# GlassyWing/yolo_deepsort

Hardware: AMD Instinct MI355X
Metric: end-to-end frames/sec (detect+ReID+assoc), 608x608 (higher is better)
Workload: dtype f16x3

## Files before the change

### include/ydsort.h

```cpp
#ifndef YDSORT_H
#define YDSORT_H

#include <stddef.h>
#include <stdint.h>

#ifdef __cplusplus
extern "C" {
#endif

typedef struct yds_net yds_net;
typedef struct yds_reid yds_reid;
typedef struct yds_trk yds_trk;
typedef struct yds_pipe yds_pipe;
typedef struct yds_comm yds_comm;

int yds_init(int device_id);
int yds_current_device(void);
int yds_device_pci_bus_id(char *buf, int len);
const char *yds_last_error(void);
int yds_device_count(void);
const char *yds_build_info(void);
void *yds_host_alloc(size_t nbytes);
int yds_host_free(void *host);
void *yds_dev_alloc(size_t nbytes);
// ... 39 lines not shown

yds_reid *yds_reid_create(int max_crops);
void yds_reid_destroy(yds_reid *);
int yds_reid_load_tensor(yds_reid *, const char *name, const float *data_host, const int64_t *shape, int ndim);
int yds_reid_finalize(yds_reid *);
int64_t yds_reid_flops_per_crop(void);
int yds_reid_embed(yds_reid *, const uint8_t *frame_rgb_host, int h, int w, const float *tlwh_host,
                   int D, float *out_host);
int yds_reid_embed_dev(yds_reid *, const uint8_t *frame_rgb_dev, int h, int w, const float *tlwh_host,
                       int D, float *out_host_or_null);
const float *yds_reid_features_dev(yds_reid *);
int yds_reid_preprocess(yds_reid *, const uint8_t *frame_rgb_host, int h, int w, const float *tlwh_host,
                        int D, float *nchw_host);
int yds_reid_preprocess_mixed(yds_reid *, const uint8_t *frames_rgb_dev, const uint64_t *frame_off, const int32_t *frame_hw ,
                              int n_frames, size_t frames_bytes, const float *tlwh_host, const int32_t *frame_of_host, int D, float *nchw_host);
int yds_reid_forward_f32(yds_reid *, const float *nchw_host, int D, float *out_host);

yds_trk *yds_tracker_create(double max_dist, double max_iou_distance, int max_age, int n_init, int nn_budget);
yds_trk *yds_tracker_create_ex(double max_dist, double max_iou_distance, int max_age, int n_init, int nn_budget, int metric);
void yds_tracker_destroy(yds_trk *);
int yds_tracker_step(yds_trk *, const float *tlwh_host, const float *feats_host, const float *payload_host,
                     int D, int32_t *out6_host, int cap, int *m_out,
                     int32_t *dbg_matches_host, int dbg_cap, int *n_matches);
int yds_tracker_step_dev(yds_trk *, const float *tlwh_host, const float *feats_dev, const float *payload_host,
                         int D, int32_t *out6_host, int cap, int *m_out);
int yds_tracker_step_sel(yds_trk *, const float *tlwh_host, const float *feats, int feats_on_device, const int32_t *feat_rows_host,
                         const float *payload_host, int D, int32_t *out6_host, int cap, int *m_out,
                         int32_t *dbg_matches_host, int dbg_cap, int *n_matches);
int yds_tracker_nms(const float *tlwh_host, const int32_t *order_host, int D, double max_overlap, int32_t *pick_host, int *n_pick);
int yds_tracker_num_tracks(const yds_trk *);
// ... 94 lines not shown
```

### yolo_deepsort_amd/_lib.py

```python

from __future__ import annotations

import ctypes as C
import os

import numpy as np

HERE = os.path.dirname(os.path.abspath(__file__))
_TAG = os.environ.get("YDS_BUILD_TAG", "")
LIB_PATH = os.path.join(HERE, "libydsort" + ("_" + _TAG if _TAG else "") + ".so")


class YdsError(RuntimeError):
    pass


_P = C.c_void_p
_I = C.c_int
_F = C.c_float
_SZ = C.c_size_t
_I64 = C.c_int64

SIGNATURES = {
    "yds_init": (_I, [_I]),
# ... 99 lines not shown
    "yds_pipeline_step_multi_host": (_I, [_P, _P, _P, _I, _I, _I, _P, _P, _I, _P]),
    "yds_pipeline_prefetch_host": (_I, [_P, _P, _I, _I, _I]),
    "yds_pipeline_set_next_injection": (_I, [_P, _I]),
    "yds_pipeline_stage_us": (_I, [_P, _P]),
    "yds_pipeline_set_schedule": (_I, [_P, _I]),
    "yds_pipeline_last_schedule": (_I, [_P]),
    "yds_pipeline_schedule_trial": (_I, [_P, _I, _P, _P, _P]),
    "yds_conv_timing": (_I, [_P, _I, _P, _P, _P]),
    "yds_overlay_tracks": (_I, [_P, _P, _I, _I, _I, _P, _P, _P, _I, _P, _P, _I, _I, _I, _P, _P]),
    "yds_swap_rb": (_I, [_P, _SZ]),
    "yds_overlay_tracks_bgr": (_I, [_P, _I, _P, _I, _I, _I, _P, _P, _P, _I, _P, _P, _I, _I, _I, _P]),
    "yds_pipeline_set_frame_order": (_I, [_P, _I]),
    "yds_pipeline_set_windows": (_I, [_P, _I, _I, C.c_double]),
    "yds_darknet_forward_u8_mixed_dev": (_I, [_P, _P, _P, _P, _SZ, _I]),
    "yds_reid_preprocess_mixed": (_I, [_P, _P, _P, _P, _I, _SZ, _P, _P, _I, _P]),
    "yds_pipeline_step_multi_mixed": (_I, [_P, _P, _P, _P, _P, _SZ, _I, _P, _P, _I, _P]),
    "yds_pipeline_step_multi_mixed_host": (_I, [_P, _P, _P, _P, _P, _SZ, _I, _P, _P, _I, _P]),
}

_lib = None
MISSING = []


def load():
    global _lib
    if _lib is not None:
        return _lib
    if not os.path.exists(LIB_PATH):
        raise YdsError(f"{LIB_PATH} not found: build it with `python -m yolo_deepsort_amd.build` "
                       "(the product has no CPU fallback)")
# ... 138 lines not shown
```

### yolo_deepsort_amd/csrc/common.h

```cpp
#pragma once
#include <hip/hip_runtime.h>
#include <stdint.h>
#include <stdio.h>
#include <string>
#include <vector>
#include <stdexcept>

namespace yds {

void set_error(const std::string &msg);
struct Error : std::runtime_error {
    explicit Error(const std::string &m) : std::runtime_error(m) {}
};
[[noreturn]] void fail(const char *fmt, ...);
int bound_device();
void bind_thread();
hipStream_t make_stream(bool latency_role);

#define YDS_HIP(expr)                                                                          \
    do {                                                                                       \
        hipError_t _e = (expr);                                                                \
        if (_e != hipSuccess)                                                                  \
            ::yds::fail("%s failed: %s (%s:%d)", #expr, hipGetErrorString(_e), __FILE__, __LINE__); \
    } while (0)
// ... 97 lines not shown
                   float logit, hipStream_t s);
void launch_inject_batch(const View &head, int batch, const float *table_dev, const int *offsets_dev, int max_rows, int head_index,
                         int num_classes, float logit, hipStream_t s);
void launch_resize_u8(const uint8_t *frames, int n, int h, int w, const View &y, hipStream_t s, bool bgr = false);
struct FrameGeom { uint64_t off; int32_t h, w; };
std::vector<FrameGeom> checked_layout(const uint64_t *frame_off, const int32_t *frame_hw, int n, size_t frames_bytes);
void launch_resize_u8_frames(const uint8_t *frames, const FrameGeom *geom, int n, const View &y, hipStream_t s, bool bgr = false);
void launch_window_resize(const uint8_t *frames, int h, int w, const int *tiles_dev, int T, int slot0, int n, const View &y, hipStream_t s,
                          bool bgr);
void launch_window_boxes(const float *pred, int n_boxes, int attrs, const int *tiles_dev, const float *scale_dev, int T, int slot0, int n,
                         float *dst, hipStream_t s);
void launch_crop_resize(const uint8_t *frames, int h, int w, const int *boxes5_dev, int D, const View &y,
                        hipStream_t s, bool bgr = false);
void launch_crop_resize_frames(const uint8_t *frames, const FrameGeom *geom, const int *boxes5_dev, int D, const View &y, hipStream_t s,
                               bool bgr = false);
void launch_avgpool_l2norm(const View &x, float *out, hipStream_t s);

}
```

### yolo_deepsort_amd/csrc/engine.h

```cpp
#pragma once
#include "common.h"

#include <map>
#include <memory>
#include <string>
#include <utility>
#include <vector>

namespace yds {

struct CfgBlock {
    std::string type;
    std::map<std::string, std::string> kv;
};
std::vector<CfgBlock> parse_cfg(const std::string &text);

struct Layer {
    std::string type;
    int c = 0, h = 0, w = 0;
    int root = -1, coff = 0;
    bool is_view = false;
    int src = -1;
    std::vector<int> refs;
    std::vector<std::pair<int, int>> copies;
// ... 138 lines not shown
    DevBuf<float> kept;
    DevBuf<int> order;
    int *h_counts = nullptr;
    float *h_kept = nullptr;
};

class ReidNet {
public:
    explicit ReidNet(int max_crops);
    ~ReidNet();
    void load_tensor(const std::string &name, const float *data, const int64_t *shape, int ndim);
    void finalize();
    void embed_dev(const uint8_t *frame_dev, int h, int w, const float *tlwh_host, int D, float *out_host);
    void embed_multi_dev(const uint8_t *frames_dev, int h, int w, const float *tlwh_host, const int *frame_of, int D, bool bgr = false,
                         const FrameGeom *geom = nullptr, int n_geom = 0);
    void crop_multi_dev(const uint8_t *frames_dev, int h, int w, const float *tlwh_host, const int *frame_of, int D, bool bgr,
                        const FrameGeom *geom, int n_geom);
    void preprocess_frames_dev(const uint8_t *frames_dev, const std::vector<FrameGeom> &geom, const float *tlwh_host, const int *frame_of, int D,
                               float *nchw_host);
    void embed_host(const uint8_t *frame_host, int h, int w, const float *tlwh_host, int D, float *out_host);
    void preprocess_host(const uint8_t *frame_host, int h, int w, const float *tlwh_host, int D, float *nchw_host);
    void forward_f32_host(const float *nchw, int D, float *out_host);
    void forward(int D);
    void reserve(int D);
    void allocate_buffers();
    static int64_t flops_per_crop();

    struct ConvW {
        int cin = 0, cin_file = 0, cout = 0, k = 0, stride = 1, pad = 0, kpad = 0;
        DevBuf<float> wt, bias;
        DevBuf<uint16_t> wt16;
    };
    int max_crops;
    std::map<std::string, std::vector<float>> raw;
    std::map<std::string, std::vector<int64_t>> raw_shape;
    bool ready = false;
    std::vector<ConvW> convs;
    std::vector<DevBuf<float>> bufs;
    DevBuf<float> in, feat, stage_f32;
    DevBuf<uint8_t> stage_u8;
    DevBuf<int> boxes_dev;
    std::vector<int> boxes_host;
    int *boxes_pin[2] = {nullptr, nullptr};
    size_t boxes_pin_cap[2] = {0, 0};
    int boxes_pin_turn = 0;
    hipStream_t sync_before_regrow = nullptr;
    std::map<int, std::pair<int, int>> tuned;
    int tuned_math = -1;
    hipStream_t stream = nullptr;
    double conv_flops_last = 0;
};

struct TrackerIface {
    virtual ~TrackerIface() {}
    virtual int step(const float *tlwh_host, const float *feats, bool feats_on_device, const float *payload_host, int D,
                     int32_t *out6_host, int cap) = 0;
    virtual int num_tracks() const = 0;
};
struct TrackerGroupIface {
    virtual ~TrackerGroupIface() {}
    virtual void step_batch(TrackerIface *const *trk, int S, int n, const int *stream_of, const float *tlwh_host, const int *first,
                            const float *feats_dev, const float *payload_host, const char *skip, int32_t *out6_host, int cap, int32_t *counts) = 0;
    virtual void wait_for(hipEvent_t ev) = 0;
};
TrackerGroupIface *make_tracker_group();
// ... 7 lines not shown
```

### yolo_deepsort_amd/csrc/layers.hip

```cpp
#include "common.h"

#include <algorithm>
#include "h16.h"

namespace yds {

static inline int grid_for(size_t work, int block = 256) {
    size_t g = (work + block - 1) / block;
    if (g > 8192) g = 8192;
    if (g < 1) g = 1;
    return (int)g;
}

__global__ void maxpool_kernel(const float *x, float *y, int N, int H, int W, int C, int ldx, int Ho, int Wo, int ldy,
                               int k, int stride, int pad, int zero_br, int fmt_in, int fmt_out) {
    fp16_saturate_on();
    const int C4 = C >> 2;
    const size_t total = (size_t)N * Ho * Wo * C4;
    for (size_t idx = blockIdx.x * (size_t)blockDim.x + threadIdx.x; idx < total; idx += (size_t)gridDim.x * blockDim.x) {
        int c4 = idx % C4;
        size_t pix = idx / C4;
        int ox = pix % Wo;
        size_t t = pix / Wo;
        int oy = t % Ho;
// ... 278 lines not shown
        else v = (t - 5 == cls) ? logit : -logit;
        cell[t] = v;
    }
}
void launch_inject_batch(const View &head, int batch, const float *table_dev, const int *offsets_dev, int max_rows, int head_index,
                         int num_classes, float logit, hipStream_t s) {
    int attrs = num_classes + 5, A = head.c / attrs;
    hipLaunchKernelGGL(inject_clear_batch_kernel, dim3(min(grid_for((size_t)head.h * head.w * A), 64), batch), dim3(256), 0, s, head.p, head.h,
                       head.w, head.ld, A, attrs, logit);
    if (max_rows > 0)
        hipLaunchKernelGGL(inject_rows_batch_kernel, dim3(max_rows, batch), dim3(128), 0, s, head.p, head.h, head.w, head.ld, attrs, table_dev,
                           offsets_dev, head_index, logit);
    YDS_HIP(hipGetLastError());
}

struct Tap { int i0, i1, a0, a1; };
__device__ __forceinline__ double cv_scale(int dst, int src) { return __ddiv_rn(1.0, __ddiv_rn((double)dst, (double)src)); }
template <bool X_AXIS> __device__ __forceinline__ Tap axis_tap(int d, double scale, int src) {
    float f = __double2float_rn(__dsub_rn(__dmul_rn((double)d + 0.5, scale), 0.5));
    const float fl = floorf(f);
    int s = (int)fl;
    f = __fsub_rn(f, fl);
    if (X_AXIS) {
        if (s < 0) { s = 0; f = 0.f; }
        if (s >= src - 1) { s = src - 1; f = 0.f; }
    }
    Tap t;
    t.a0 = (int)rintf(__fmul_rn(__fsub_rn(1.f, f), 2048.f));
    t.a1 = (int)rintf(__fmul_rn(f, 2048.f));
    t.i0 = min(max(s, 0), src - 1);
    t.i1 = min(max(s + 1, 0), src - 1);
    return t;
}
enum { RESIZE_LINEAR = 0, RESIZE_AREA2 = 1, RESIZE_COPY = 2 };
__device__ __forceinline__ int resize_mode(int src_h, int src_w, int dst_h, int dst_w) {
    if (src_h == dst_h && src_w == dst_w) return RESIZE_COPY;
    if (src_h == 2 * dst_h && src_w == 2 * dst_w) return RESIZE_AREA2;
    return RESIZE_LINEAR;
}
__device__ __forceinline__ void resize_px(const uint8_t *base, size_t row_bytes, int src_h, int src_w, int dst_h, int dst_w, int oy, int ox,
                                          float o[3]) {
    const int mode = resize_mode(src_h, src_w, dst_h, dst_w);
    if (mode == RESIZE_COPY) {
        const uint8_t *p = base + (size_t)oy * row_bytes + ox * 3;
        o[0] = p[0]; o[1] = p[1]; o[2] = p[2];
        return;
    }
    if (mode == RESIZE_AREA2) {
        const uint8_t *p = base + (size_t)(2 * oy) * row_bytes + 2 * ox * 3, *q = p + row_bytes;
#pragma unroll
        for (int c = 0; c < 3; ++c) o[c] = (float)(((int)p[c] + (int)p[3 + c] + (int)q[c] + (int)q[3 + c] + 2) >> 2);
        return;
    }
    const Tap tx = axis_tap<true>(ox, cv_scale(dst_w, src_w), src_w), ty = axis_tap<false>(oy, cv_scale(dst_h, src_h), src_h);
    const uint8_t *r0 = base + (size_t)ty.i0 * row_bytes, *r1 = base + (size_t)ty.i1 * row_bytes;
#pragma unroll
    for (int c = 0; c < 3; ++c) {
        const int h0 = (int)r0[tx.i0 * 3 + c] * tx.a0 + (int)r0[tx.i1 * 3 + c] * tx.a1;
        const int h1 = (int)r1[tx.i0 * 3 + c] * tx.a0 + (int)r1[tx.i1 * 3 + c] * tx.a1;
        o[c] = (float)(((((ty.a0 * (h0 >> 4)) >> 16) + ((ty.a1 * (h1 >> 4)) >> 16) + 2) >> 2) & 0xff);
    }
}

__global__ void resize_u8_kernel(const uint8_t *frames, int N, int H, int W, float *y, int Ho, int Wo, int ldy, int bgr) {
    const size_t total = (size_t)N * Ho * Wo;
    for (size_t idx = blockIdx.x * (size_t)blockDim.x + threadIdx.x; idx < total; idx += (size_t)gridDim.x * blockDim.x) {
        int ox = idx % Wo;
        size_t t = idx / Wo;
        int oy = t % Ho;
        int n = t / Ho;
        float o[3];
        resize_px(frames + (size_t)n * H * W * 3, (size_t)W * 3, H, W, Ho, Wo, oy, ox, o);
        if (bgr) { const float t = o[0]; o[0] = o[2]; o[2] = t; }
        *reinterpret_cast<float4 *>(y + idx * ldy) = make_float4(__fdiv_rn(o[0], 255.f), __fdiv_rn(o[1], 255.f), __fdiv_rn(o[2], 255.f), 0.f);
    }
}

// ... 168 lines not shown
```

### yolo_deepsort_amd/csrc/reid.cpp

```cpp
#include "engine.h"
#include "h16.h"

#include <math.h>
#include <stdlib.h>
#include <string.h>

namespace yds {

namespace {
struct StageDef { const char *name; int cin, cout; bool down; };
const StageDef kStages[4] = {{"layer1", 64, 64, false}, {"layer2", 64, 128, true}, {"layer3", 128, 256, true}, {"layer4", 256, 512, true}};
constexpr int CROP_H = 128, CROP_W = 64, EMB = 512;
}

ReidNet::ReidNet(int max_crops) : max_crops(max_crops) {
    if (max_crops < 1) fail("reid: max_crops must be positive");
    stream = make_stream(false);
}
ReidNet::~ReidNet() {
    if (stream) { (void)hipStreamSynchronize(stream); (void)hipStreamDestroy(stream); }
    for (int *b : boxes_pin) if (b) (void)hipHostFree(b);
}

void ReidNet::load_tensor(const std::string &name, const float *data, const int64_t *shape, int ndim) {
// ... 60 lines not shown
    for (const StageDef &s : kStages) {
        for (int b = 0; b < 2; ++b) {
            std::string p = std::string(s.name) + "." + std::to_string(b);
            int ci = b == 0 ? s.cin : s.cout;
            bool down = b == 0 && s.down;
            add_conv(p + ".conv1", p + ".bn1", ci, s.cout, 3, down ? 2 : 1, false);
            add_conv(p + ".conv2", p + ".bn2", s.cout, s.cout, 3, 1, false);
            if (down) add_conv(p + ".downsample.0", p + ".downsample.1", ci, s.cout, 1, 2, false);
        }
    }
    allocate_buffers();
    ready = true;
}

void ReidNet::allocate_buffers() {
    in.alloc((size_t)max_crops * CROP_H * CROP_W * 4);
    feat.alloc((size_t)max_crops * EMB);
    bufs.clear();
    bufs.emplace_back((size_t)max_crops * CROP_H * CROP_W * 64);
    bufs.emplace_back((size_t)max_crops * 64 * 32 * 64);
    int h = 64, w = 32;
    for (const StageDef &s : kStages) {
        if (s.down) { h /= 2; w /= 2; }
        for (int k = 0; k < 5; ++k) bufs.emplace_back((size_t)max_crops * h * w * s.cout);
    }
}

void ReidNet::reserve(int D) {
    if (D <= max_crops) return;
    YDS_HIP(hipStreamSynchronize(stream));
    int m = max_crops;
    while (m < D) m *= 2;
    max_crops = m;
    if (ready) allocate_buffers();
    else in.alloc((size_t)max_crops * CROP_H * CROP_W * 4);
}

void ReidNet::forward(int D) {
    if (!ready) fail("reid: weights not loaded (yds_reid_finalize)");
    if (D < 1) fail("reid: no crops");
    reserve(D);
    const bool f16 = conv_math() == MATH_F16X3;
    auto mk = [&](DevBuf<float> &b, int h, int w, int c) {
        View v; v.p = b.p; v.n = D; v.h = h; v.w = w; v.c = c; v.ld = c;
        v.fmt = (f16 && c % 32 == 0) ? FMT_H16 : FMT_F32;
        return v;
    };
    conv_flops_last = 0;
    auto run = [&](int ci, const View &x, const View &y, int act, const View *res, int res_mode) {
        const ConvW &c = convs[ci];
        ConvArgs a;
        a.x = x; a.y = y; a.w = c.wt.p; a.w16 = c.wt16.p; a.bias = c.bias.p;
        a.ksize = c.k; a.stride = c.stride; a.pad = c.pad; a.kpad = c.kpad; a.act = act;
        if (res) { a.res = *res; a.res_mode = res_mode; }
        if (tuned_math != conv_math()) { tuned.clear(); tuned_math = conv_math(); }
        auto it = tuned.find(ci);
        if (it == tuned.end() || D > 2 * it->second.first || 2 * D < it->second.first) {
            int v = conv_autotune(a, stream, nullptr);
            tuned[ci] = std::make_pair(D, v);
            it = tuned.find(ci);
        }
        (void)launch_conv(a, stream, it->second.second);
        conv_flops_last += conv_flops(a);
    };
    View x0 = mk(in, CROP_H, CROP_W, 4);
    View cur = mk(bufs[1], 64, 32, 64);
    {
        const ConvW &c = convs[0];
        ConvArgs a;
        a.x = x0; a.y = cur; a.w = c.wt.p; a.w16 = c.wt16.p; a.bias = c.bias.p;
        a.ksize = c.k; a.stride = c.stride; a.pad = c.pad; a.kpad = c.kpad; a.act = ACT_RELU;
        if (!getenv("YDS_REID_UNFUSED") && launch_conv_maxpool3s2(a, stream)) {
            conv_flops_last += 2.0 * D * CROP_H * CROP_W * 64 * 9 * 4;
        } else {
            View stem = mk(bufs[0], CROP_H, CROP_W, 64);
            run(0, x0, stem, ACT_RELU, nullptr, RES_NONE);
            launch_maxpool(stem, cur, 3, 2, 1, false, stream);
        }
    }
    int ci = 1, bi = 2, h = 64, w = 32;
    for (const StageDef &s : kStages) {
        if (s.down) { h /= 2; w /= 2; }
        for (int b = 0; b < 2; ++b) {
            bool down = b == 0 && s.down;
            View y1 = mk(bufs[bi + (b == 0 ? 0 : 3)], h, w, s.cout);
            View out = mk(bufs[bi + (b == 0 ? 1 : 4)], h, w, s.cout);
            run(ci, cur, y1, ACT_RELU, nullptr, RES_NONE);
            View res = cur;
            if (down) {
// ... 27 lines not shown
            fail("reid: detection %d yields an empty crop (%d,%d,%d,%d) in frame %d (%d x %d); cv2.resize raises in the reference", d, x1, y1, x2, y2,
                 frame_of[d], H, W);
        if (x2 <= x1 || y2 <= y1) fail("reid: detection %d yields an empty crop (%d,%d,%d,%d); cv2.resize raises in the reference", d, x1, y1, x2, y2);
        out[d * 5] = x1; out[d * 5 + 1] = y1; out[d * 5 + 2] = x2; out[d * 5 + 3] = y2; out[d * 5 + 4] = frame_of ? frame_of[d] : 0;
    }
}

void ReidNet::embed_dev(const uint8_t *frame_dev, int h, int w, const float *tlwh_host, int D, float *out_host) {
    if (D == 0) return;
    if (!ready) fail("reid: weights not loaded (yds_reid_finalize)");
    reserve(D);
    std::vector<int> boxes;
    crop_boxes_host(tlwh_host, D, h, w, boxes);
    boxes_dev.upload(boxes.data(), boxes.size(), stream);
    YDS_HIP(hipStreamSynchronize(stream));
    View x0; x0.p = in.p; x0.n = D; x0.h = CROP_H; x0.w = CROP_W; x0.c = 4; x0.ld = 4;
    launch_crop_resize(frame_dev, h, w, boxes_dev.p, D, x0, stream);
    forward(D);
    if (out_host) YDS_HIP(hipMemcpyAsync(out_host, feat.p, (size_t)D * EMB * sizeof(float), hipMemcpyDeviceToHost, stream));
    YDS_HIP(hipStreamSynchronize(stream));
}

void ReidNet::embed_multi_dev(const uint8_t *frames_dev, int h, int w, const float *tlwh_host, const int *frame_of, int D, bool bgr,
                              const FrameGeom *geom, int n_geom) {
    if (D == 0) return;
    if (!ready) fail("reid: weights not loaded (yds_reid_finalize)");
    crop_multi_dev(frames_dev, h, w, tlwh_host, frame_of, D, bgr, geom, n_geom);
    forward(D);
}

void ReidNet::crop_multi_dev(const uint8_t *frames_dev, int h, int w, const float *tlwh_host, const int *frame_of, int D, bool bgr,
                             const FrameGeom *geom, int n_geom) {
    reserve(D);
    crop_boxes_host(tlwh_host, D, h, w, boxes_host, frame_of, geom, n_geom);
    static_assert(sizeof(FrameGeom) == 4 * sizeof(int), "the frame table is laid out in the int list");
    const size_t head = geom ? (size_t)n_geom * 4 : 0, need = head + boxes_host.size();
    const int t = boxes_pin_turn ^= 1;
    if (boxes_pin_cap[t] < need) {
        if (boxes_pin[t]) {
            YDS_HIP(hipStreamSynchronize(stream));
            if (sync_before_regrow) YDS_HIP(hipStreamSynchronize(sync_before_regrow));
            (void)hipHostFree(boxes_pin[t]);
            boxes_pin[t] = nullptr;
        }
        boxes_pin_cap[t] = std::max<size_t>(need * 2, 4096);
        YDS_HIP(hipHostMalloc((void **)&boxes_pin[t], boxes_pin_cap[t] * sizeof(int), hipHostMallocDefault));
    }
    if (geom) memcpy(boxes_pin[t], geom, head * sizeof(int));
    memcpy(boxes_pin[t] + head, boxes_host.data(), boxes_host.size() * sizeof(int));
    View x0; x0.p = in.p; x0.n = D; x0.h = CROP_H; x0.w = CROP_W; x0.c = 4; x0.ld = 4;
    if (geom) launch_crop_resize_frames(frames_dev, reinterpret_cast<const FrameGeom *>(boxes_pin[t]), boxes_pin[t] + head, D, x0, stream, bgr);
    else launch_crop_resize(frames_dev, h, w, boxes_pin[t], D, x0, stream, bgr);
}

void ReidNet::preprocess_frames_dev(const uint8_t *frames_dev, const std::vector<FrameGeom> &geom, const float *tlwh_host, const int *frame_of,
                                    int D, float *nchw_host) {
    if (D == 0) return;
    reserve(D);
    if (!in.p) in.alloc((size_t)max_crops * CROP_H * CROP_W * 4);
    crop_multi_dev(frames_dev, 0, 0, tlwh_host, frame_of, D, false, geom.data(), (int)geom.size());
    View x3; x3.p = in.p; x3.n = D; x3.h = CROP_H; x3.w = CROP_W; x3.c = 3; x3.ld = 4;
    DevBuf<float> tmp((size_t)D * 3 * CROP_H * CROP_W);
    launch_nhwc_to_nchw(x3, tmp.p, stream);
    YDS_HIP(hipMemcpyAsync(nchw_host, tmp.p, tmp.n * sizeof(float), hipMemcpyDeviceToHost, stream));
    YDS_HIP(hipStreamSynchronize(stream));
}

void ReidNet::embed_host(const uint8_t *frame_host, int h, int w, const float *tlwh_host, int D, float *out_host) {
    size_t n = (size_t)h * w * 3;
    stage_u8.ensure(n);
    YDS_HIP(hipMemcpyAsync(stage_u8.p, frame_host, n, hipMemcpyHostToDevice, stream));
    embed_dev(stage_u8.p, h, w, tlwh_host, D, out_host);
    YDS_HIP(hipStreamSynchronize(stream));
}

void ReidNet::preprocess_host(const uint8_t *frame_host, int h, int w, const float *tlwh_host, int D, float *nchw_host) {
    if (D == 0) return;
    reserve(D);
    if (!in.p) in.alloc((size_t)max_crops * CROP_H * CROP_W * 4);
    size_t n = (size_t)h * w * 3;
    stage_u8.ensure(n);
    YDS_HIP(hipMemcpyAsync(stage_u8.p, frame_host, n, hipMemcpyHostToDevice, stream));
    std::vector<int> boxes;
    crop_boxes_host(tlwh_host, D, h, w, boxes);
    boxes_dev.upload(boxes.data(), boxes.size(), stream);
    YDS_HIP(hipStreamSynchronize(stream));
    View x0; x0.p = in.p; x0.n = D; x0.h = CROP_H; x0.w = CROP_W; x0.c = 4; x0.ld = 4;
    launch_crop_resize(stage_u8.p, h, w, boxes_dev.p, D, x0, stream);
    View x3 = x0; x3.c = 3;
    DevBuf<float> tmp((size_t)D * 3 * CROP_H * CROP_W);
    launch_nhwc_to_nchw(x3, tmp.p, stream);
    YDS_HIP(hipMemcpyAsync(nchw_host, tmp.p, tmp.n * sizeof(float), hipMemcpyDeviceToHost, stream));
    YDS_HIP(hipStreamSynchronize(stream));
}

void ReidNet::forward_f32_host(const float *nchw, int D, float *out_host) {
    if (D == 0) return;
    if (!ready) fail("reid: weights not loaded (yds_reid_finalize)");
    reserve(D);
    size_t n = (size_t)D * 3 * CROP_H * CROP_W;
    stage_f32.ensure(n);
    YDS_HIP(hipMemcpyAsync(stage_f32.p, nchw, n * sizeof(float), hipMemcpyHostToDevice, stream));
    View x0; x0.p = in.p; x0.n = D; x0.h = CROP_H; x0.w = CROP_W; x0.c = 4; x0.ld = 4;
    launch_nchw_to_nhwc(stage_f32.p, x0, 3, stream);
    forward(D);
    YDS_HIP(hipMemcpyAsync(out_host, feat.p, (size_t)D * EMB * sizeof(float), hipMemcpyDeviceToHost, stream));
    YDS_HIP(hipStreamSynchronize(stream));
}

}


extern "C" {

yds_reid *yds_reid_create(int max_crops) {
    YDS_API_BEGIN
    return new yds_reid{new yds::ReidNet(max_crops)};
    YDS_API_END_PTR
// ... 23 lines not shown
    YDS_API_END
}
const float *yds_reid_features_dev(yds_reid *r) { return r->r->feat.p; }
int yds_reid_preprocess(yds_reid *r, const uint8_t *frame, int h, int w, const float *tlwh, int D, float *nchw) {
    YDS_API_BEGIN
    r->r->preprocess_host(frame, h, w, tlwh, D, nchw);
    YDS_API_END
}
int yds_reid_preprocess_mixed(yds_reid *r, const uint8_t *frames_dev, const uint64_t *frame_off, const int32_t *frame_hw, int n_frames,
                              size_t frames_bytes, const float *tlwh, const int32_t *frame_of, int D, float *nchw) {
    YDS_API_BEGIN
    if (!frames_dev) yds::fail("reid: NULL frames");
    r->r->preprocess_frames_dev(frames_dev, yds::checked_layout(frame_off, frame_hw, n_frames, frames_bytes), tlwh, frame_of, D, nchw);
    YDS_API_END
}
int yds_reid_forward_f32(yds_reid *r, const float *nchw, int D, float *out) {
    YDS_API_BEGIN
    r->r->forward_f32_host(nchw, D, out);
    YDS_API_END
}

}
```

### yolo_deepsort_amd/deep_sort.py

```python

from __future__ import annotations

import ctypes as C

import numpy as np

from . import _lib
from .loaders import load_reid_checkpoint

__all__ = ["DeepSort", "Extractor", "build_tracker"]


def _np(x, dtype=np.float32):
    if hasattr(x, "detach"):
        x = x.detach().cpu().numpy()
    return np.ascontiguousarray(x, dtype=dtype)


class Extractor:

    def __init__(self, model_path, use_cuda=True, max_crops=256):
        _lib.init()
        lib = _lib.load()
        self.device = "cuda"
# ... 31 lines not shown

    def preprocess_mixed(self, frames, tlwh, frame_of):
        from .pipeline import pack_frames
        block, off, hw = pack_frames(frames)
        tlwh = _np(tlwh).reshape(-1, 4)
        frame_of = np.ascontiguousarray(frame_of, dtype=np.int32).reshape(-1)
        assert frame_of.size == tlwh.shape[0]
        out = np.empty((tlwh.shape[0], 3, 128, 64), np.float32)
        dev = _lib.DeviceBuffer.from_array(block)
        try:
            _lib.check(_lib.load().yds_reid_preprocess_mixed(self._h, dev.ptr, _lib.ptr(off), _lib.ptr(hw), len(off), block.nbytes,
                                                             _lib.ptr(tlwh), _lib.ptr(frame_of), tlwh.shape[0], _lib.ptr(out)))
        finally:
            dev.free()
        return out

    def forward(self, batch):
        batch = _np(batch)
        out = np.empty((batch.shape[0], 512), np.float32)
        _lib.check(_lib.load().yds_reid_forward_f32(self._h, _lib.ptr(batch), batch.shape[0], _lib.ptr(out)))
        return out

    def features_dev(self):
        return _lib.load().yds_reid_features_dev(self._h)

    def __call__(self, im_crops):
        if len(im_crops) == 0:
            return np.zeros((0, 512), np.float32)
        wmax = max(c.shape[1] for c in im_crops)
        htot = sum(c.shape[0] for c in im_crops)
# ... 174 lines not shown
```

Baseline: 1612.

## Fuse ReID crop-resize, stem conv and maxpool into one MFMA kernel

Adds a persistent ReID stem kernel that samples each crop straight from the frames with bilinear resize, runs the 3x3 stem conv on split-f16 MFMA, and applies ReLU plus 3x3/s2 max pooling before writing the pooled H16 activations. This removes the separate crop-resize kernel and the full-resolution 128x64 input buffer round trip through global memory. The unfused path stays available behind environment variables, buffers are now allocated lazily, and a new mixed-frame embed API is exposed. Risks are numeric differences from the split-precision conv and the complexity of the hand-written kernel.

```diff
diff --git a/include/ydsort.h b/include/ydsort.h
--- a/include/ydsort.h
+++ b/include/ydsort.h
@@ -77,6 +77,11 @@
                         int D, float *nchw_host);
 int yds_reid_preprocess_mixed(yds_reid *, const uint8_t *frames_rgb_dev, const uint64_t *frame_off, const int32_t *frame_hw ,
                               int n_frames, size_t frames_bytes, const float *tlwh_host, const int32_t *frame_of_host, int D, float *nchw_host);
+int yds_reid_embed_mixed(yds_reid *, const uint8_t *frames_dev, const uint64_t *frame_off, const int32_t *frame_hw ,
+                         int n_frames, size_t frames_bytes, const float *tlwh_host, const int32_t *frame_of_host, int D, int bgr,
+                         float *out_host);
+int yds_reid_front_fused(yds_reid *);
+int yds_reid_front_grid_crops(void);
 int yds_reid_forward_f32(yds_reid *, const float *nchw_host, int D, float *out_host);
 
 yds_trk *yds_tracker_create(double max_dist, double max_iou_distance, int max_age, int n_init, int nn_budget);
diff --git a/yolo_deepsort_amd/_lib.py b/yolo_deepsort_amd/_lib.py
--- a/yolo_deepsort_amd/_lib.py
+++ b/yolo_deepsort_amd/_lib.py
@@ -137,6 +137,9 @@
     "yds_pipeline_set_windows": (_I, [_P, _I, _I, C.c_double]),
     "yds_darknet_forward_u8_mixed_dev": (_I, [_P, _P, _P, _P, _SZ, _I]),
     "yds_reid_preprocess_mixed": (_I, [_P, _P, _P, _P, _I, _SZ, _P, _P, _I, _P]),
+    "yds_reid_embed_mixed": (_I, [_P, _P, _P, _P, _I, _SZ, _P, _P, _I, _I, _P]),
+    "yds_reid_front_fused": (_I, [_P]),
+    "yds_reid_front_grid_crops": (_I, []),
     "yds_pipeline_step_multi_mixed": (_I, [_P, _P, _P, _P, _P, _SZ, _I, _P, _P, _I, _P]),
     "yds_pipeline_step_multi_mixed_host": (_I, [_P, _P, _P, _P, _P, _SZ, _I, _P, _P, _I, _P]),
 }
diff --git a/yolo_deepsort_amd/csrc/common.h b/yolo_deepsort_amd/csrc/common.h
--- a/yolo_deepsort_amd/csrc/common.h
+++ b/yolo_deepsort_amd/csrc/common.h
@@ -135,6 +135,15 @@
                         hipStream_t s, bool bgr = false);
 void launch_crop_resize_frames(const uint8_t *frames, const FrameGeom *geom, const int *boxes5_dev, int D, const View &y, hipStream_t s,
                                bool bgr = false);
+struct ReidFront {
+    const uint8_t *frames = nullptr;
+    const FrameGeom *geom = nullptr;
+    const int *boxes = nullptr;
+    int h = 0, w = 0, bgr = 0;
+};
+void launch_reid_stem(const ReidFront &f, int D, const float *w, int kpad, const float *bias, const View &pooled, hipStream_t s);
+constexpr int kReidStemUnitsPerCrop = 4;
+int reid_stem_grid();
 void launch_avgpool_l2norm(const View &x, float *out, hipStream_t s);
 
 }
diff --git a/yolo_deepsort_amd/csrc/engine.h b/yolo_deepsort_amd/csrc/engine.h
--- a/yolo_deepsort_amd/csrc/engine.h
+++ b/yolo_deepsort_amd/csrc/engine.h
@@ -176,15 +176,17 @@
     void embed_dev(const uint8_t *frame_dev, int h, int w, const float *tlwh_host, int D, float *out_host);
     void embed_multi_dev(const uint8_t *frames_dev, int h, int w, const float *tlwh_host, const int *frame_of, int D, bool bgr = false,
                          const FrameGeom *geom = nullptr, int n_geom = 0);
-    void crop_multi_dev(const uint8_t *frames_dev, int h, int w, const float *tlwh_host, const int *frame_of, int D, bool bgr,
-                        const FrameGeom *geom, int n_geom);
     void preprocess_frames_dev(const uint8_t *frames_dev, const std::vector<FrameGeom> &geom, const float *tlwh_host, const int *frame_of, int D,
                                float *nchw_host);
     void embed_host(const uint8_t *frame_host, int h, int w, const float *tlwh_host, int D, float *out_host);
     void preprocess_host(const uint8_t *frame_host, int h, int w, const float *tlwh_host, int D, float *nchw_host);
     void forward_f32_host(const float *nchw, int D, float *out_host);
-    void forward(int D);
+    void forward(int D, const ReidFront *front = nullptr);
     void reserve(int D);
+    float *in_buf();
+    void crop_into_in(const ReidFront &f, int D);
+    ReidFront stage_crops(const uint8_t *frames_dev, int h, int w, const float *tlwh_host, const int *frame_of, int D, bool bgr,
+                          const FrameGeom *geom, int n_geom);
     void allocate_buffers();
     static int64_t flops_per_crop();
 
@@ -211,6 +213,7 @@
     int tuned_math = -1;
     hipStream_t stream = nullptr;
     double conv_flops_last = 0;
+    bool front_fused_last = false;
 };
 
 struct TrackerIface {
diff --git a/yolo_deepsort_amd/csrc/layers.hip b/yolo_deepsort_amd/csrc/layers.hip
--- a/yolo_deepsort_amd/csrc/layers.hip
+++ b/yolo_deepsort_amd/csrc/layers.hip
@@ -2,6 +2,7 @@
 
 #include <algorithm>
 #include "h16.h"
+#include "resize_dev.h"
 
 namespace yds {
 
@@ -316,53 +317,6 @@
     YDS_HIP(hipGetLastError());
 }
 
-struct Tap { int i0, i1, a0, a1; };
-__device__ __forceinline__ double cv_scale(int dst, int src) { return __ddiv_rn(1.0, __ddiv_rn((double)dst, (double)src)); }
-template <bool X_AXIS> __device__ __forceinline__ Tap axis_tap(int d, double scale, int src) {
-    float f = __double2float_rn(__dsub_rn(__dmul_rn((double)d + 0.5, scale), 0.5));
-    const float fl = floorf(f);
-    int s = (int)fl;
-    f = __fsub_rn(f, fl);
-    if (X_AXIS) {
-        if (s < 0) { s = 0; f = 0.f; }
-        if (s >= src - 1) { s = src - 1; f = 0.f; }
-    }
-    Tap t;
-    t.a0 = (int)rintf(__fmul_rn(__fsub_rn(1.f, f), 2048.f));
-    t.a1 = (int)rintf(__fmul_rn(f, 2048.f));
-    t.i0 = min(max(s, 0), src - 1);
-    t.i1 = min(max(s + 1, 0), src - 1);
-    return t;
-}
-enum { RESIZE_LINEAR = 0, RESIZE_AREA2 = 1, RESIZE_COPY = 2 };
-__device__ __forceinline__ int resize_mode(int src_h, int src_w, int dst_h, int dst_w) {
-    if (src_h == dst_h && src_w == dst_w) return RESIZE_COPY;
-    if (src_h == 2 * dst_h && src_w == 2 * dst_w) return RESIZE_AREA2;
-    return RESIZE_LINEAR;
-}
-__device__ __forceinline__ void resize_px(const uint8_t *base, size_t row_bytes, int src_h, int src_w, int dst_h, int dst_w, int oy, int ox,
-                                          float o[3]) {
-    const int mode = resize_mode(src_h, src_w, dst_h, dst_w);
-    if (mode == RESIZE_COPY) {
-        const uint8_t *p = base + (size_t)oy * row_bytes + ox * 3;
-        o[0] = p[0]; o[1] = p[1]; o[2] = p[2];
-        return;
-    }
-    if (mode == RESIZE_AREA2) {
-        const uint8_t *p = base + (size_t)(2 * oy) * row_bytes + 2 * ox * 3, *q = p + row_bytes;
-#pragma unroll
-        for (int c = 0; c < 3; ++c) o[c] = (float)(((int)p[c] + (int)p[3 + c] + (int)q[c] + (int)q[3 + c] + 2) >> 2);
-        return;
-    }
-    const Tap tx = axis_tap<true>(ox, cv_scale(dst_w, src_w), src_w), ty = axis_tap<false>(oy, cv_scale(dst_h, src_h), src_h);
-    const uint8_t *r0 = base + (size_t)ty.i0 * row_bytes, *r1 = base + (size_t)ty.i1 * row_bytes;
-#pragma unroll
-    for (int c = 0; c < 3; ++c) {
-        const int h0 = (int)r0[tx.i0 * 3 + c] * tx.a0 + (int)r0[tx.i1 * 3 + c] * tx.a1;
-        const int h1 = (int)r1[tx.i0 * 3 + c] * tx.a0 + (int)r1[tx.i1 * 3 + c] * tx.a1;
-        o[c] = (float)(((((ty.a0 * (h0 >> 4)) >> 16) + ((ty.a1 * (h1 >> 4)) >> 16) + 2) >> 2) & 0xff);
-    }
-}
 
 __global__ void resize_u8_kernel(const uint8_t *frames, int N, int H, int W, float *y, int Ho, int Wo, int ldy, int bgr) {
     const size_t total = (size_t)N * Ho * Wo;
diff --git a/yolo_deepsort_amd/csrc/reid.cpp b/yolo_deepsort_amd/csrc/reid.cpp
--- a/yolo_deepsort_amd/csrc/reid.cpp
+++ b/yolo_deepsort_amd/csrc/reid.cpp
@@ -98,10 +98,9 @@
 }
 
 void ReidNet::allocate_buffers() {
-    in.alloc((size_t)max_crops * CROP_H * CROP_W * 4);
     feat.alloc((size_t)max_crops * EMB);
     bufs.clear();
-    bufs.emplace_back((size_t)max_crops * CROP_H * CROP_W * 64);
+    bufs.emplace_back();
     bufs.emplace_back((size_t)max_crops * 64 * 32 * 64);
     int h = 64, w = 32;
     for (const StageDef &s : kStages) {
@@ -117,10 +116,20 @@
     while (m < D) m *= 2;
     max_crops = m;
     if (ready) allocate_buffers();
-    else in.alloc((size_t)max_crops * CROP_H * CROP_W * 4);
-}
-
-void ReidNet::forward(int D) {
+}
+
+float *ReidNet::in_buf() {
+    in.ensure((size_t)max_crops * CROP_H * CROP_W * 4);
+    return in.p;
+}
+
+void ReidNet::crop_into_in(const ReidFront &f, int D) {
+    View x0; x0.p = in_buf(); x0.n = D; x0.h = CROP_H; x0.w = CROP_W; x0.c = 4; x0.ld = 4;
+    if (f.geom) launch_crop_resize_frames(f.frames, f.geom, f.boxes, D, x0, stream, f.bgr);
+    else launch_crop_resize(f.frames, f.h, f.w, f.boxes, D, x0, stream, f.bgr);
+}
+
+void ReidNet::forward(int D, const ReidFront *front) {
     if (!ready) fail("reid: weights not loaded (yds_reid_finalize)");
     if (D < 1) fail("reid: no crops");
     reserve(D);
@@ -147,9 +156,18 @@
         (void)launch_conv(a, stream, it->second.second);
         conv_flops_last += conv_flops(a);
     };
-    View x0 = mk(in, CROP_H, CROP_W, 4);
     View cur = mk(bufs[1], 64, 32, 64);
-    {
+    const bool fused_front = front && f16 && cur.fmt == FMT_H16 && !getenv("YDS_POOL_VALU") && !getenv("YDS_REID_UNFUSED") &&
+                             !getenv("YDS_REID_FRONT_UNFUSED");
+    front_fused_last = fused_front;
+    if (fused_front) {
+        const ConvW &c = convs[0];
+        launch_reid_stem(*front, D, c.wt.p, c.kpad, c.bias.p, cur, stream);
+        conv_flops_last += 2.0 * D * CROP_H * CROP_W * 64 * 9 * 4;
+    } else {
+        if (front) crop_into_in(*front, D);
+        in_buf();
+        View x0 = mk(in, CROP_H, CROP_W, 4);
         const ConvW &c = convs[0];
         ConvArgs a;
         a.x = x0; a.y = cur; a.w = c.wt.p; a.w16 = c.wt16.p; a.bias = c.bias.p;
@@ -157,6 +175,7 @@
         if (!getenv("YDS_REID_UNFUSED") && launch_conv_maxpool3s2(a, stream)) {
             conv_flops_last += 2.0 * D * CROP_H * CROP_W * 64 * 9 * 4;
         } else {
+            bufs[0].ensure((size_t)max_crops * CROP_H * CROP_W * 64);
             View stem = mk(bufs[0], CROP_H, CROP_W, 64);
             run(0, x0, stem, ACT_RELU, nullptr, RES_NONE);
             launch_maxpool(stem, cur, 3, 2, 1, false, stream);
@@ -214,9 +233,9 @@
     crop_boxes_host(tlwh_host, D, h, w, boxes);
     boxes_dev.upload(boxes.data(), boxes.size(), stream);
     YDS_HIP(hipStreamSynchronize(stream));
-    View x0; x0.p = in.p; x0.n = D; x0.h = CROP_H; x0.w = CROP_W; x0.c = 4; x0.ld = 4;
-    launch_crop_resize(frame_dev, h, w, boxes_dev.p, D, x0, stream);
-    forward(D);
+    ReidFront front;
+    front.frames = frame_dev; front.h = h; front.w = w; front.boxes = boxes_dev.p;
+    forward(D, &front);
     if (out_host) YDS_HIP(hipMemcpyAsync(out_host, feat.p, (size_t)D * EMB * sizeof(float), hipMemcpyDeviceToHost, stream));
     YDS_HIP(hipStreamSynchronize(stream));
 }
@@ -225,12 +244,12 @@
                               const FrameGeom *geom, int n_geom) {
     if (D == 0) return;
     if (!ready) fail("reid: weights not loaded (yds_reid_finalize)");
-    crop_multi_dev(frames_dev, h, w, tlwh_host, frame_of, D, bgr, geom, n_geom);
-    forward(D);
-}
-
-void ReidNet::crop_multi_dev(const uint8_t *frames_dev, int h, int w, const float *tlwh_host, const int *frame_of, int D, bool bgr,
-                             const FrameGeom *geom, int n_geom) {
+    const ReidFront front = stage_crops(frames_dev, h, w, tlwh_host, frame_of, D, bgr, geom, n_geom);
+    forward(D, &front);
+}
+
+ReidFront ReidNet::stage_crops(const uint8_t *frames_dev, int h, int w, const float *tlwh_host, const int *frame_of, int D, bool bgr,
+                               const FrameGeom *geom, int n_geom) {
     reserve(D);
     crop_boxes_host(tlwh_host, D, h, w, boxes_host, frame_of, geom, n_geom);
     static_assert(sizeof(FrameGeom) == 4 * sizeof(int), "the frame table is laid out in the int list");
@@ -248,17 +267,17 @@
     }
     if (geom) memcpy(boxes_pin[t], geom, head * sizeof(int));
     memcpy(boxes_pin[t] + head, boxes_host.data(), boxes_host.size() * sizeof(int));
-    View x0; x0.p = in.p; x0.n = D; x0.h = CROP_H; x0.w = CROP_W; x0.c = 4; x0.ld = 4;
-    if (geom) launch_crop_resize_frames(frames_dev, reinterpret_cast<const FrameGeom *>(boxes_pin[t]), boxes_pin[t] + head, D, x0, stream, bgr);
-    else launch_crop_resize(frames_dev, h, w, boxes_pin[t], D, x0, stream, bgr);
+    ReidFront front;
+    front.frames = frames_dev; front.h = h; front.w = w; front.bgr = bgr ? 1 : 0;
+    front.geom = geom ? reinterpret_cast<const FrameGeom *>(boxes_pin[t]) : nullptr;
+    front.boxes = boxes_pin[t] + head;
+    return front;
 }
 
 void ReidNet::preprocess_frames_dev(const uint8_t *frames_dev, const std::vector<FrameGeom> &geom, const float *tlwh_host, const int *frame_of,
                                     int D, float *nchw_host) {
     if (D == 0) return;
-    reserve(D);
-    if (!in.p) in.alloc((size_t)max_crops * CROP_H * CROP_W * 4);
-    crop_multi_dev(frames_dev, 0, 0, tlwh_host, frame_of, D, false, geom.data(), (int)geom.size());
+    crop_into_in(stage_crops(frames_dev, 0, 0, tlwh_host, frame_of, D, false, geom.data(), (int)geom.size()), D);
     View x3; x3.p = in.p; x3.n = D; x3.h = CROP_H; x3.w = CROP_W; x3.c = 3; x3.ld = 4;
     DevBuf<float> tmp((size_t)D * 3 * CROP_H * CROP_W);
     launch_nhwc_to_nchw(x3, tmp.p, stream);
@@ -277,7 +296,6 @@
 void ReidNet::preprocess_host(const uint8_t *frame_host, int h, int w, const float *tlwh_host, int D, float *nchw_host) {
     if (D == 0) return;
     reserve(D);
-    if (!in.p) in.alloc((size_t)max_crops * CROP_H * CROP_W * 4);
     size_t n = (size_t)h * w * 3;
     stage_u8.ensure(n);
     YDS_HIP(hipMemcpyAsync(stage_u8.p, frame_host, n, hipMemcpyHostToDevice, stream));
@@ -285,7 +303,7 @@
     crop_boxes_host(tlwh_host, D, h, w, boxes);
     boxes_dev.upload(boxes.data(), boxes.size(), stream);
     YDS_HIP(hipStreamSynchronize(stream));
-    View x0; x0.p = in.p; x0.n = D; x0.h = CROP_H; x0.w = CROP_W; x0.c = 4; x0.ld = 4;
+    View x0; x0.p = in_buf(); x0.n = D; x0.h = CROP_H; x0.w = CROP_W; x0.c = 4; x0.ld = 4;
     launch_crop_resize(stage_u8.p, h, w, boxes_dev.p, D, x0, stream);
     View x3 = x0; x3.c = 3;
     DevBuf<float> tmp((size_t)D * 3 * CROP_H * CROP_W);
@@ -301,7 +319,7 @@
     size_t n = (size_t)D * 3 * CROP_H * CROP_W;
     stage_f32.ensure(n);
     YDS_HIP(hipMemcpyAsync(stage_f32.p, nchw, n * sizeof(float), hipMemcpyHostToDevice, stream));
-    View x0; x0.p = in.p; x0.n = D; x0.h = CROP_H; x0.w = CROP_W; x0.c = 4; x0.ld = 4;
+    View x0; x0.p = in_buf(); x0.n = D; x0.h = CROP_H; x0.w = CROP_W; x0.c = 4; x0.ld = 4;
     launch_nchw_to_nhwc(stage_f32.p, x0, 3, stream);
     forward(D);
     YDS_HIP(hipMemcpyAsync(out_host, feat.p, (size_t)D * EMB * sizeof(float), hipMemcpyDeviceToHost, stream));
@@ -355,6 +373,24 @@
     r->r->preprocess_frames_dev(frames_dev, yds::checked_layout(frame_off, frame_hw, n_frames, frames_bytes), tlwh, frame_of, D, nchw);
     YDS_API_END
 }
+int yds_reid_embed_mixed(yds_reid *r, const uint8_t *frames_dev, const uint64_t *frame_off, const int32_t *frame_hw, int n_frames,
+                         size_t frames_bytes, const float *tlwh, const int32_t *frame_of, int D, int bgr, float *out) {
+    YDS_API_BEGIN
+    if (!frames_dev) yds::fail("reid: NULL frames");
+    if (D < 1) return 0;
+    const std::vector<yds::FrameGeom> geom = yds::checked_layout(frame_off, frame_hw, n_frames, frames_bytes);
+    yds::ReidNet &net = *r->r;
+    net.embed_multi_dev(frames_dev, 0, 0, tlwh, frame_of, D, bgr != 0, geom.data(), (int)geom.size());
+    YDS_HIP(hipMemcpyAsync(out, net.feat.p, (size_t)D * 512 * sizeof(float), hipMemcpyDeviceToHost, net.stream));
+    YDS_HIP(hipStreamSynchronize(net.stream));
+    YDS_API_END
+}
+int yds_reid_front_fused(yds_reid *r) { return r && r->r->front_fused_last ? 1 : 0; }
+int yds_reid_front_grid_crops(void) {
+    YDS_API_BEGIN
+    return yds::reid_stem_grid() / yds::kReidStemUnitsPerCrop;
+    YDS_API_END
+}
 int yds_reid_forward_f32(yds_reid *r, const float *nchw, int D, float *out) {
     YDS_API_BEGIN
     r->r->forward_f32_host(nchw, D, out);
diff --git a/yolo_deepsort_amd/csrc/reid_stem.hip b/yolo_deepsort_amd/csrc/reid_stem.hip
--- /dev/null
+++ b/yolo_deepsort_amd/csrc/reid_stem.hip
@@ -0,0 +1,211 @@
+#include "conv_common.h"
+#include "resize_dev.h"
+
+#include <algorithm>
+
+namespace yds {
+
+namespace {
+constexpr int RS_H = 128, RS_W = 64, RS_HP = 64, RS_WP = 32;
+constexpr int RS_PR = 16, RS_WR = 8;
+constexpr int RS_UNITS = RS_HP / RS_PR;
+static_assert(RS_UNITS == kReidStemUnitsPerCrop, "common.h tells the callers");
+constexpr int RS_IR = 2 * RS_PR + 3;
+constexpr int RS_PW = RS_W / 2 + 1, RS_ROW = 2 * RS_PW;
+constexpr int RS_NT = 256, RS_OCC = 3;
+static_assert(RS_NT / 64 == 2 * (RS_PR / RS_WR), "one wave per channel half and 8 pooled rows");
+
+struct CropSrc { unsigned long long off; int row_bytes, cw, ch, pad; };
+
+__device__ __forceinline__ float rs_max(float a, float b) {
+    float r;
+    asm("v_max_f32 %0, %1, %2" : "=v"(r) : "v"(a), "v"(b));
+    return r;
+}
+__device__ __forceinline__ float rs_max3(float a, float b, float c) {
+    float r;
+    asm("v_max3_f32 %0, %1, %2, %3" : "=v"(r) : "v"(a), "v"(b), "v"(c));
+    return r;
+}
+
+__device__ __forceinline__ int rs_entry(int c) { return (c & 1) ? (c + 1) >> 1 : RS_PW + (c >> 1); }
+}
+
+__global__ __launch_bounds__(RS_NT, RS_OCC) void reid_stem_kernel(ReidFront f, const float *w, int kpad, const float *bias, float *y, int n_units) {
+    fp16_saturate_on();
+    __shared__ __attribute__((aligned(16))) h16x4 tile_hi[RS_IR * RS_ROW], tile_lo[RS_IR * RS_ROW];
+    __shared__ CropSrc src[2];
+    __shared__ unsigned int norm[3 * 256];
+    const int tid = threadIdx.x, lane = tid & 63, wave = tid >> 6, kb = lane >> 5, j = lane & 31, n = wave & 1, sub = wave >> 1;
+    h8 wh[3], wl[3];
+#pragma unroll
+    for (int sb = 0; sb < 3; ++sb)
+#pragma unroll
+        for (int e = 0; e < 8; ++e) {
+            const int t = 4 * sb + 2 * kb + (e >> 2), c = e & 3;
+            const float x = (t < 9 && c < 3) ? w[(size_t)(n * 32 + j) * kpad + t * 4 + c] : 0.f;
+            const _Float16 h = (_Float16)x;
+            wh[sb][e] = h;
+            wl[sb][e] = (_Float16)((x - (float)h) * 2048.f);
+        }
+    int off[2][3][2];
+#pragma unroll
+    for (int fr = 0; fr < 2; ++fr)
+#pragma unroll
+        for (int sb = 0; sb < 3; ++sb)
+#pragma unroll
+            for (int h = 0; h < 2; ++h) {
+                const int t = 4 * sb + 2 * kb + h;
+                off[fr][sb][h] = t < 9 ? (t / 3) * RS_ROW + rs_entry(2 * j + fr - 1 + t % 3) : 0;
+            }
+    for (int i = tid; i < 3 * 256; i += RS_NT) {
+        const float mean[3] = {0.485f, 0.456f, 0.406f}, stdv[3] = {0.229f, 0.224f, 0.225f};
+        const int c = i >> 8;
+        const float px[4] = {__fdiv_rn(__fsub_rn(__fdiv_rn((float)(i & 255), 255.f), mean[c]), stdv[c]), 0.f, 0.f, 0.f};
+        union { h16x4 h; unsigned short u[4]; } hi, lo;
+        h16_encode4(px, hi.h, lo.h);
+        norm[i] = hi.u[0] | (unsigned int)lo.u[0] << 16;
+    }
+    auto load_src = [&](int u, int slot) {
+        const int *b = f.boxes + (size_t)(u / RS_UNITS) * 5;
+        const int x1 = b[0], y1 = b[1], x2 = b[2], y2 = b[3], fi = b[4];
+        CropSrc c;
+        if (f.geom) {
+            const FrameGeom g = f.geom[fi];
+            c.off = g.off + ((unsigned long long)y1 * g.w + x1) * 3;
+            c.row_bytes = g.w * 3;
+        } else {
+            c.off = ((unsigned long long)fi * f.h * f.w + (unsigned long long)y1 * f.w + x1) * 3;
+            c.row_bytes = f.w * 3;
+        }
+        c.cw = x2 - x1; c.ch = y2 - y1; c.pad = 0;
+        src[slot] = c;
+    };
+    if (tid == 0) load_src(blockIdx.x, 0);
+    int cur = 0;
+    for (int u = blockIdx.x; u < n_units; u += gridDim.x, cur ^= 1) {
+        __syncthreads();
+        if (tid == 0 && u + (int)gridDim.x < n_units) load_src(u + gridDim.x, cur ^ 1);
+        const CropSrc cs = src[cur];
+        const int d = u / RS_UNITS, py0 = (u - d * RS_UNITS) * RS_PR, iy0 = 2 * py0 - 2;
+        const uint8_t *base = f.frames + cs.off;
+        const int ix = tid & (RS_W - 1);
+        for (int r = tid / RS_W; r < RS_IR; r += RS_NT / RS_W) {
+            const int iy = iy0 + r;
+            uint2 vh = make_uint2(0u, 0u), vl = make_uint2(0u, 0u);
+            if ((unsigned)iy < (unsigned)RS_H) {
+                float o[3];
+                resize_px(base, (size_t)cs.row_bytes, cs.ch, cs.cw, RS_H, RS_W, iy, ix, o);
+                if (f.bgr) { const float t = o[0]; o[0] = o[2]; o[2] = t; }
+                const unsigned int e0 = norm[(int)o[0]], e1 = norm[256 + (int)o[1]], e2 = norm[512 + (int)o[2]];
+                vh = make_uint2((e0 & 0xffffu) | e1 << 16, e2 & 0xffffu);
+                vl = make_uint2(e0 >> 16 | (e1 & 0xffff0000u), e2 >> 16);
+            }
+            *reinterpret_cast<uint2 *>(&tile_hi[r * RS_ROW + rs_entry(ix)]) = vh;
+            *reinterpret_cast<uint2 *>(&tile_lo[r * RS_ROW + rs_entry(ix)]) = vl;
+        }
+        if (tid < 2 * RS_IR) {
+            const int e = (tid >> 1) * RS_ROW + ((tid & 1) ? RS_ROW - 1 : 0);
+            tile_hi[e] = h16x4{0, 0, 0, 0};
+            tile_lo[e] = h16x4{0, 0, 0, 0};
+        }
+        __syncthreads();
+        auto conv_row = [&](int r, float hm[16]) {
+            const int row = (r + 1 - 2 * py0) * RS_ROW;
+            float t[2][16];
+#pragma unroll
+            for (int fr = 0; fr < 2; ++fr) {
+                f32x16 c1, c2;
+#pragma unroll
+                for (int e = 0; e < 16; ++e) { c1[e] = 0.f; c2[e] = 0.f; }
+#pragma unroll
+                for (int sb = 0; sb < 3; ++sb) {
+                    union { h16x4 q[2]; h8 v; } xh, xl;
+#pragma unroll
+                    for (int h = 0; h < 2; ++h) {
+                        xh.q[h] = tile_hi[row + off[fr][sb][h]];
+                        xl.q[h] = tile_lo[row + off[fr][sb][h]];
+                    }
+                    c1 = __builtin_amdgcn_mfma_f32_32x32x16_f16(wh[sb], xh.v, c1, 0, 0, 0);
+                    c2 = __builtin_amdgcn_mfma_f32_32x32x16_f16(wh[sb], xl.v, c2, 0, 0, 0);
+                    c2 = __builtin_amdgcn_mfma_f32_32x32x16_f16(wl[sb], xh.v, c2, 0, 0, 0);
+                }
+#pragma unroll
+                for (int e = 0; e < 16; ++e) t[fr][e] = c1[e] + c2[e] * (1.f / 2048.f);
+            }
+#pragma unroll
+            for (int e = 0; e < 16; ++e) {
+                const int own = __float_as_int(t[1][e]), left = __builtin_amdgcn_update_dpp(own, own, 0x138, 0xF, 0xF, false);
+                hm[e] = rs_max3(t[0][e], t[1][e], __int_as_float(j == 0 ? own : left));
+            }
+        };
+        const int p0 = py0 + sub * RS_WR;
+        float run[16];
+#pragma unroll 1
+        for (int i = 0; i <= 2 * RS_WR; ++i) {
+            const int r = 2 * p0 - 1 + i, Py = r >> 1;
+            float hm[16];
+            conv_row(r, hm);
+            if (r & 1) {
+                if (i == 0) {
+#pragma unroll
+                    for (int e = 0; e < 16; ++e) run[e] = r < 0 ? -INFINITY : hm[e];
+                    continue;
+                }
+            } else {
+#pragma unroll
+                for (int e = 0; e < 16; ++e) run[e] = rs_max(run[e], hm[e]);
+                continue;
+            }
+            union { h16x4 h; unsigned int i[2]; } hi[4], lo[4];
+#pragma unroll
+            for (int g = 0; g < 4; ++g) {
+                const float4 b4 = *reinterpret_cast<const float4 *>(bias + n * 32 + 8 * g + 4 * kb);
+                const float bb[4] = {b4.x, b4.y, b4.z, b4.w};
+                float m[4];
+#pragma unroll
+                for (int c = 0; c < 4; ++c) {
+                    m[c] = apply_act<ACT_RELU>(rs_max(run[g * 4 + c], hm[g * 4 + c]) * 256.f + bb[c]);
+                    run[g * 4 + c] = hm[g * 4 + c];
+                }
+                h16_encode4(m, hi[g].h, lo[g].h);
+            }
+            char *pix = reinterpret_cast<char *>(y + ((size_t)(d * RS_HP + Py) * RS_WP + j) * 64) + n * 128 + kb * 16;
+#pragma unroll
+            for (int p = 0; p < 2; ++p) {
+#pragma unroll
+                for (int l = 0; l < 2; ++l) {
+                    unsigned int *ka = l ? lo[2 * p].i : hi[2 * p].i, *kn = l ? lo[2 * p + 1].i : hi[2 * p + 1].i;
+                    const auto s0 = __builtin_amdgcn_permlane32_swap(ka[0], kn[0], false, false);
+                    const auto s1 = __builtin_amdgcn_permlane32_swap(ka[1], kn[1], false, false);
+                    uint4 o4;
+                    o4.x = s0[0]; o4.y = s1[0]; o4.z = s0[1]; o4.w = s1[1];
+                    *reinterpret_cast<uint4 *>(pix + l * 64 + p * 32) = o4;
+                }
+            }
+        }
+    }
+}
+
+int reid_stem_grid() {
+    static int grid = 0;
+    if (!grid) {
+        int dev = 0, cus = 0;
+        YDS_HIP(hipGetDevice(&dev));
+        YDS_HIP(hipDeviceGetAttribute(&cus, hipDeviceAttributeMultiprocessorCount, dev));
+        grid = std::max(cus, 1) * RS_OCC;
+    }
+    return grid;
+}
+
+void launch_reid_stem(const ReidFront &f, int D, const float *w, int kpad, const float *bias, const View &pooled, hipStream_t s) {
+    if (D < 1) return;
+    if (pooled.fmt != FMT_H16 || pooled.h != RS_HP || pooled.w != RS_WP || pooled.c != 64 || pooled.ld != 64 || pooled.n < D)
+        fail("reid stem: the pooled view must be H16 [D,%d,%d,64]", RS_HP, RS_WP);
+    if (!f.frames || !f.boxes) fail("reid stem: no frames or no crop list");
+    const int n_units = D * RS_UNITS;
+    hipLaunchKernelGGL(reid_stem_kernel, dim3((unsigned)std::min(n_units, reid_stem_grid())), dim3(RS_NT), 0, s, f, w, kpad, bias, pooled.p, n_units);
+    YDS_HIP(hipGetLastError());
+}
+
+}
diff --git a/yolo_deepsort_amd/csrc/resize_dev.h b/yolo_deepsort_amd/csrc/resize_dev.h
--- /dev/null
+++ b/yolo_deepsort_amd/csrc/resize_dev.h
@@ -0,0 +1,55 @@
+#pragma once
+#include <hip/hip_runtime.h>
+#include <stdint.h>
+
+namespace yds {
+
+struct Tap { int i0, i1, a0, a1; };
+__device__ __forceinline__ double cv_scale(int dst, int src) { return __ddiv_rn(1.0, __ddiv_rn((double)dst, (double)src)); }
+template <bool X_AXIS> __device__ __forceinline__ Tap axis_tap(int d, double scale, int src) {
+    float f = __double2float_rn(__dsub_rn(__dmul_rn((double)d + 0.5, scale), 0.5));
+    const float fl = floorf(f);
+    int s = (int)fl;
+    f = __fsub_rn(f, fl);
+    if (X_AXIS) {
+        if (s < 0) { s = 0; f = 0.f; }
+        if (s >= src - 1) { s = src - 1; f = 0.f; }
+    }
+    Tap t;
+    t.a0 = (int)rintf(__fmul_rn(__fsub_rn(1.f, f), 2048.f));
+    t.a1 = (int)rintf(__fmul_rn(f, 2048.f));
+    t.i0 = min(max(s, 0), src - 1);
+    t.i1 = min(max(s + 1, 0), src - 1);
+    return t;
+}
+enum { RESIZE_LINEAR = 0, RESIZE_AREA2 = 1, RESIZE_COPY = 2 };
+__device__ __forceinline__ int resize_mode(int src_h, int src_w, int dst_h, int dst_w) {
+    if (src_h == dst_h && src_w == dst_w) return RESIZE_COPY;
+    if (src_h == 2 * dst_h && src_w == 2 * dst_w) return RESIZE_AREA2;
+    return RESIZE_LINEAR;
+}
+__device__ __forceinline__ void resize_px(const uint8_t *base, size_t row_bytes, int src_h, int src_w, int dst_h, int dst_w, int oy, int ox,
+                                          float o[3]) {
+    const int mode = resize_mode(src_h, src_w, dst_h, dst_w);
+    if (mode == RESIZE_COPY) {
+        const uint8_t *p = base + (size_t)oy * row_bytes + ox * 3;
+        o[0] = p[0]; o[1] = p[1]; o[2] = p[2];
+        return;
+    }
+    if (mode == RESIZE_AREA2) {
+        const uint8_t *p = base + (size_t)(2 * oy) * row_bytes + 2 * ox * 3, *q = p + row_bytes;
+#pragma unroll
+        for (int c = 0; c < 3; ++c) o[c] = (float)(((int)p[c] + (int)p[3 + c] + (int)q[c] + (int)q[3 + c] + 2) >> 2);
+        return;
+    }
+    const Tap tx = axis_tap<true>(ox, cv_scale(dst_w, src_w), src_w), ty = axis_tap<false>(oy, cv_scale(dst_h, src_h), src_h);
+    const uint8_t *r0 = base + (size_t)ty.i0 * row_bytes, *r1 = base + (size_t)ty.i1 * row_bytes;
+#pragma unroll
+    for (int c = 0; c < 3; ++c) {
+        const int h0 = (int)r0[tx.i0 * 3 + c] * tx.a0 + (int)r0[tx.i1 * 3 + c] * tx.a1;
+        const int h1 = (int)r1[tx.i0 * 3 + c] * tx.a0 + (int)r1[tx.i1 * 3 + c] * tx.a1;
+        o[c] = (float)(((((ty.a0 * (h0 >> 4)) >> 16) + ((ty.a1 * (h1 >> 4)) >> 16) + 2) >> 2) & 0xff);
+    }
+}
+
+}
diff --git a/yolo_deepsort_amd/deep_sort.py b/yolo_deepsort_amd/deep_sort.py
--- a/yolo_deepsort_amd/deep_sort.py
+++ b/yolo_deepsort_amd/deep_sort.py
@@ -69,6 +69,24 @@
         finally:
             dev.free()
         return out
+
+    def embed_mixed(self, frames, tlwh, frame_of, bgr=False):
+        from .pipeline import pack_frames
+        block, off, hw = pack_frames(frames)
+        tlwh = _np(tlwh).reshape(-1, 4)
+        frame_of = np.ascontiguousarray(frame_of, dtype=np.int32).reshape(-1)
+        assert frame_of.size == tlwh.shape[0]
+        out = np.empty((tlwh.shape[0], 512), np.float32)
+        dev = _lib.DeviceBuffer.from_array(block)
+        try:
+            _lib.check(_lib.load().yds_reid_embed_mixed(self._h, dev.ptr, _lib.ptr(off), _lib.ptr(hw), len(off), block.nbytes,
+                                                        _lib.ptr(tlwh), _lib.ptr(frame_of), tlwh.shape[0], 1 if bgr else 0, _lib.ptr(out)))
+        finally:
+            dev.free()
+        return out
+
+    def front_fused(self):
+        return bool(_lib.load().yds_reid_front_fused(self._h))
 
     def forward(self, batch):
         batch = _np(batch)
```

After: 1635 (median of 6 runs). 1.4% higher.
